# nlapier2/Metalign

Measured on NVIDIA B200. Metric: read k-mers/sec queried vs CMash DB, higher is better.
Workload: dtype u128

## Files before the change

metalign_b200/csrc/probe_mz.cu:

```cuda
#ifdef MZ_RT
#define MLG_RT MZ_RT
#endif
#include "probe_common.cuh"

namespace {

#ifndef MZ_MINCTAS
#define MZ_MINCTAS 2
#endif
constexpr unsigned MZ_MAXRUN = 4;
constexpr unsigned MZ_QDRAIN = 32;
constexpr unsigned MZ_QCAP = MZ_QDRAIN + 128;
constexpr unsigned MZ_LIST = 16;
constexpr uint32_t MZ_M64 = MLG_MZ_ORD_MULT << 6;
#ifndef MZ_TILE_READS
#define MZ_TILE_READS 32
#endif
constexpr unsigned MZ_TR = MZ_TILE_READS;
static_assert(MZ_TR % 32 == 0 && MZ_TR >= 32 && MZ_TR <= 128, "tile = whole warp passes");
constexpr unsigned MZ_STAGE_B = MZ_TR * 40 + 64;
constexpr unsigned MZ_STAGE_M = MZ_TR * 20 + 64;
struct MzStage {
    __align__(16) unsigned char b[WARPS][2][MZ_STAGE_B];
    __align__(16) unsigned char m[WARPS][2][MZ_STAGE_M];
};
struct MzShared {
    MzStage stg;
    uint32_t wm[MZ_LIST][RT];
    uint32_t seq[SEGW + 1][RT];
    uint32_t qa[WARPS][MZ_QCAP];
    uint32_t qc[WARPS][MZ_QCAP];
    uint32_t qb[WARPS][MZ_QCAP];
    uint32_t qoff[WARPS][32];
    uint32_t qn[WARPS];
};
constexpr uint32_t MZ_ROW = RT * 4;

#ifndef MZ_L2_FETCH
#define MZ_L2_FETCH 64
#endif
#if MZ_L2_FETCH == 64
#define MZ_L2Q ".L2::64B"
#elif MZ_L2_FETCH == 128
#define MZ_L2Q ".L2::128B"
#else
#define MZ_L2Q ""
#endif
__device__ __forceinline__ uint32_t ldg_bitmap_if(bool p, const uint32_t* ptr) {
    uint32_t r;
    asm volatile(
        "{\n"
        ".reg .pred q;\n"
        "setp.ne.u32 q, %1, 0;\n"
        "mov.u32 %0, 0;\n"
        "@q ld.global.nc.L1::no_allocate" MZ_L2Q ".b32 %0, [%2];\n"
        "}\n" : "=r"(r) : "r"((uint32_t)p), "l"(ptr));
    return r;
}
__device__ __forceinline__ uint32_t ldg_u32(const uint32_t* ptr) {
    uint32_t r;
    asm volatile("ld.global.nc" MZ_L2Q ".b32 %0, [%1];" : "=r"(r) : "l"(ptr));
    return r;
}
__device__ __forceinline__ key128 ldg_key(const key128* ptr) {
    key128 k;
    asm volatile("ld.global.nc" MZ_L2Q ".v2.u64 {%0, %1}, [%2];" : "=l"(k.hi), "=l"(k.lo) : "l"(ptr));
    return k;
}
template <bool HAS_NMASK>
__device__ __forceinline__ void segment_load_staged(uint32_t (&loc)[SEGW], uint32_t (&nl)[5], uint32_t brel, uint32_t mrel, uint32_t sb, uint32_t sk) {
    const uint32_t ab = sb + (brel >> 4) * 4u;
    const unsigned sh = 2u * (brel & 15u);
    uint32_t W[SEGW + 1];
#pragma unroll
    for (int k = 0; k <= (int)SEGW; ++k) W[k] = __byte_perm(lds32(ab + 4u * (uint32_t)k), 0, 0x0123);
#pragma unroll
    for (int k = 0; k < (int)SEGW; ++k) loc[k] = fsl(W[k], W[k + 1], sh);
#pragma unroll
    for (int k = 0; k < 5; ++k) nl[k] = 0;
    if (HAS_NMASK) {
        const uint32_t am = sk + (mrel >> 5) * 4u;
        const unsigned shn = mrel & 31u;
        uint32_t M[6];
#pragma unroll
        for (int k = 0; k < 6; ++k) M[k] = __byte_perm(lds32(am + 4u * (uint32_t)k), 0, 0x0123);
#pragma unroll
        for (int k = 0; k < 5; ++k) nl[k] = fsl(M[k], M[k + 1], shn);
    }
}
__device__ __forceinline__ uint32_t mz_val(const uint32_t (&loc)[SEGW], const uint32_t (&rcl)[SEGW], int j, int i) {
    const uint32_t a = fsl(loc[j], loc[j + 1], 2 * i);
    const int ra = i <= 11 ? 7 - j : 6 - j, ro = i <= 11 ? 11 - i : 27 - i;
    const uint32_t b = fsl(rcl[ra], rcl[ra + 1], 2 * ro);
    return b * MZ_M64 + (a * MZ_M64 + (uint32_t)(16 * j + i));
}
__device__ __forceinline__ void mz_bases64(const unsigned long long* bsrc, unsigned long long base_words, unsigned long long p,
                                           unsigned long long& hi, unsigned long long& lo) {
    const unsigned long long q = p >> 5;
    const unsigned sh = 2u * (unsigned)(p & 31ull);
    unsigned long long W[3];
#pragma unroll
    for (int k = 0; k < 3; ++k) {
        unsigned long long idx = q + k;
        if (idx >= base_words) idx = base_words - 1;
        W[k] = bswap64(bsrc[idx]);
    }
    hi = sh ? ((W[0] << sh) | (W[1] >> (64 - sh))) : W[0];
    lo = sh ? ((W[1] << sh) | (W[2] >> (64 - sh))) : W[1];
}
struct MzWin {
    key128 cn, d0, d1;
    uint32_t s, e, j0, j1;
};
__device__ __forceinline__ void mz_window_begin(MzWin& w, bool on, unsigned long long p, unsigned long long pm,
                                                const unsigned long long* bsrc, unsigned long long base_words, const DbView& db) {
    w.s = w.e = w.j0 = w.j1 = 0;
    w.cn.hi = w.cn.lo = 0; w.d0 = w.cn; w.d1 = w.cn;
    if (!on) return;
    key128 F;
    mz_bases64(bsrc, base_words, p, F.hi, F.lo);
    const unsigned dsh = 2u * (unsigned)(pm - p);
    const unsigned long long mh = dsh ? ((F.hi << dsh) | (F.lo >> (64u - dsh))) : F.hi;
    const uint32_t ha = (uint32_t)(mh >> 32), hb = rev2_32(~(uint32_t)mh);
    const uint32_t zhi = mz_ident_hi(ha, hb), zlo = mz_ident_lo(ha, hb);
    const uint32_t bucket = zhi >> (32u - db.bbits);
    w.s = ldg_u32(db.bstart + bucket); w.e = ldg_u32(db.bstart + bucket + 1);
    if (db.n_alias && ((db.alias_bloom[(zlo & 0xFFFFu) >> 5] >> (zlo & 31u)) & 1u)) {
        const unsigned long long z = ((unsigned long long)zhi << 32) | zlo;
        uint32_t lo = 0, hi = db.n_alias;
        while (lo < hi) { const uint32_t mid = (lo + hi) >> 1; if (db.alias_z[mid] < z) lo = mid + 1; else hi = mid; }
        w.j0 = w.j1 = lo;
        while (w.j1 < db.n_alias && db.alias_z[w.j1] == z) ++w.j1;
    }
    F = key_shr(F, 128 - 2 * SK_K);
    const key128 G = key_rc(F, SK_K);
    w.cn = key_lt(G, F) ? G : F;
    if (w.s < w.e) w.d0 = ldg_key(db.D_key + w.s);
    if (w.s + 1u < w.e) w.d1 = ldg_key(db.D_key + w.s + 1u);
}
__device__ __forceinline__ void mz_window_end(const MzWin& w, const DbView& db, const CountSink& cs) {
    if (w.s < w.e && w.d0.hi == w.cn.hi && w.d0.lo == w.cn.lo) { bump_counter(cs, w.s); return; }
    if (w.s + 1u < w.e && w.d1.hi == w.cn.hi && w.d1.lo == w.cn.lo) { bump_counter(cs, w.s + 1u); return; }
    for (uint32_t i = w.s + 2u; i < w.e; ++i) {
        const key128 d = ldg_key(db.D_key + i);
        if (d.hi == w.cn.hi && d.lo == w.cn.lo) { bump_counter(cs, i); return; }
    }
    for (uint32_t j = w.j0; j < w.j1; ++j) {
        const uint32_t i = db.alias_i[j];
        const key128 d = db.D_key[i];
        if (d.hi == w.cn.hi && d.lo == w.cn.lo) { bump_counter(cs, i); return; }
    }
}
__device__ __noinline__ void mz_drain(uint32_t* qn, const uint32_t* qa, const uint32_t* qc, uint32_t* qb, uint32_t* qoff,
                                      const ProbeArgs& a, const DbView& db) {
    const unsigned long long* const bsrc = a.bases;
    const unsigned long long base_words = a.base_words;
    const CountSink cs{a.cnt8, a.present, a.n_present, a.touched, a.ci_min};
    constexpr unsigned FULL = 0xFFFFFFFFu;
    const unsigned lane = threadIdx.x & 31u;
    __syncwarp();
    const uint32_t n = *qn;
    for (uint32_t base = 0; base < n; base += 32u) {
        const uint32_t i = base + lane;
        uint32_t kb0 = i < n ? qb[i] : 0u;
        if (__any_sync(FULL, (kb0 >> 31) != 0u)) {
            if (kb0 >> 31) {
                const unsigned long long pb = ((unsigned long long)qc[i] << 32) | qa[i];
                unsigned long long mh, ml;
                mz_bases64(bsrc, base_words, pb + ((kb0 >> 16) & 63u), mh, ml);
                const uint32_t ha = (uint32_t)(mh >> 32), hb = rev2_32(~(uint32_t)mh);
                const uint32_t zhi = mz_ident_hi(ha, hb), zlo = mz_ident_lo(ha, hb);
                const unsigned long long idx = mz_bit_index(((unsigned long long)zhi << 32) | zlo, db.fbits);
                const uint32_t f = ldg_u32(db.F + (idx >> 5));
                kb0 = ((f >> (zlo & 31u)) & (f >> mz_bit2(zhi)) & 1u) ? (kb0 & 0x7FFFFFFFu) : 0u;
                qb[i] = kb0;
            }
            __syncwarp();
        }
        const uint32_t cnt = (uint32_t)__popc(kb0 & 0xFFFFu);
        uint32_t inc = cnt;
#pragma unroll
        for (int o = 1; o < 32; o <<= 1) { const uint32_t u = __shfl_up_sync(FULL, inc, o); if ((int)lane >= o) inc += u; }
        const uint32_t total = __shfl_sync(FULL, inc, 31);
        qoff[lane] = inc - cnt;
        __syncwarp();
        for (uint32_t w = lane; w < total; w += 32u) {
            uint32_t j = 0;
#pragma unroll
            for (uint32_t step = 16; step; step >>= 1) if (qoff[j + step] <= w) j += step;
            const uint32_t kb = qb[base + j];
            const uint32_t tt = __fns(kb & 0xFFFFu, 0u, (int)(w - qoff[j]) + 1);
            const unsigned long long pb = ((unsigned long long)qc[base + j] << 32) | qa[base + j];
            MzWin win;
            mz_window_begin(win, true, pb + tt, pb + ((kb >> 16) & 63u), bsrc, base_words, db);
            mz_window_end(win, db, cs);
        }
        __syncwarp();
    }
    __syncwarp();
    if (lane == 0) *qn = 0;
    __syncwarp();
}

template <bool HAS_NMASK>
__global__ void __launch_bounds__(RT, MZ_MINCTAS) k1_minimizer_probe(const __grid_constant__ ProbeArgs a, const __grid_constant__ DbView db) {
    extern __shared__ __align__(16) unsigned char smem_raw[];
    MzShared& sm = *reinterpret_cast<MzShared*>(smem_raw);
    MzStage& stg = sm.stg;
    __shared__ __align__(8) unsigned long long mbar[WARPS][2];
    __shared__ unsigned long long s_bw0[WARPS][2], s_mw0[WARPS][2];
    __shared__ unsigned s_staged[WARPS][2];
    __shared__ __align__(16) uint32_t s_zero[SEGW + 2];

    const unsigned tid = threadIdx.x, warp = tid >> 5, lane = tid & 31u;
    constexpr unsigned K = SK_K;
    if (tid < SEGW + 2) s_zero[tid] = 0u;
    constexpr unsigned FULL = 0xFFFFFFFFu;
    const unsigned long long nreads = a.r_end - a.r_begin;
    const unsigned long long ntiles = (nreads + MZ_TR - 1) / MZ_TR;
    unsigned int* const tile_ctr = reinterpret_cast<unsigned int*>(a.tile_counter);
    auto next_tile = [&]() -> unsigned long long {
        unsigned int t = 0;
        if (lane == 0) t = atomicAdd(tile_ctr, 1u);
        return __shfl_sync(FULL, t, 0);
    };
#ifdef MZ_STREAM_EVICT_FIRST
    const unsigned long long pol_stream = policy_evict_first();
#elif defined(MZ_STREAM_EVICT_LAST)
    const unsigned long long pol_stream = policy_evict_last();
#else
    unsigned long long pol_stream;
    asm volatile("createpolicy.fractional.L2::evict_normal.b64 %0, 1.0;" : "=l"(pol_stream));
#endif
    const uint32_t wm_base = smem_u32(&sm.wm[0][tid]), seq_base = smem_u32(&sm.seq[0][tid]);
    const uint32_t* const MB = db.F;
    const uint32_t lt_mask = (1u << lane) - 1u;
    const uint32_t fmask_lo = db.fbits >= 32u ? 0xFFFFFFFFu : ((1u << db.fbits) - 1u);
    const uint32_t fmask_hi = db.fbits > 32u ? ((1u << (db.fbits - 32u)) - 1u) : 0u;

    if (lane == 0) {
        mbar_init(&mbar[warp][0], 1);
        mbar_init(&mbar[warp][1], 1);
        asm volatile("fence.mbarrier_init.release.cluster;" ::: "memory");
    }
    __syncthreads();

    auto issue = [&](unsigned stage, unsigned long long t) {
        const unsigned long long r0 = a.r_begin + t * (unsigned long long)MZ_TR;
        const unsigned long long r1 = (r0 + MZ_TR < a.r_end) ? r0 + MZ_TR : a.r_end;
        const unsigned long long p0 = a.off ? a.off[r0] : r0 * (unsigned long long)a.read_len;
        const unsigned long long p1 = a.off ? a.off[r1] : r1 * (unsigned long long)a.read_len;
        unsigned long long bw0 = (p0 >> 5) & ~1ull;
        unsigned long long bw1 = ((p1 + 31) >> 5) + 6;
        if (bw1 > a.base_words) bw1 = a.base_words;
        bw1 = (bw1 + 1) & ~1ull;
        unsigned long long mw0 = (p0 >> 6) & ~1ull;
        unsigned long long mw1 = ((p1 + 63) >> 6) + 4;
        if (HAS_NMASK) { if (mw1 > a.nmask_words) mw1 = a.nmask_words; mw1 = (mw1 + 1) & ~1ull; }
        const unsigned long long bytes_b = (bw1 - bw0) * 8ull, bytes_m = HAS_NMASK ? (mw1 - mw0) * 8ull : 0ull;
        const bool fits = bw1 > bw0 && bytes_b <= MZ_STAGE_B && bytes_m <= MZ_STAGE_M;
        s_bw0[warp][stage] = bw0; s_mw0[warp][stage] = mw0; s_staged[warp][stage] = fits ? 1u : 0u;
        if (fits) {
            mbar_expect_tx(&mbar[warp][stage], (uint32_t)(bytes_b + bytes_m));
            bulk_g2s(&stg.b[warp][stage][0], a.bases + bw0, (uint32_t)bytes_b, &mbar[warp][stage], pol_stream);
            if (HAS_NMASK && bytes_m) bulk_g2s(&stg.m[warp][stage][0], a.nmask + mw0, (uint32_t)bytes_m, &mbar[warp][stage], pol_stream);
        } else {
            mbar_arrive(&mbar[warp][stage]);
        }
    };

    unsigned my_valid = 0;
    unsigned my_fetch = 0;
    if (lane == 0) sm.qn[warp] = 0;
    __syncwarp();

    auto halves_at = [&](uint32_t P, uint32_t& ha, uint32_t& hb) {
        const uint32_t ad = seq_base + (P >> 4) * MZ_ROW;
        const uint32_t w0 = lds32(ad), w1 = lds32(ad + MZ_ROW), w2 = lds32(ad + 2u * MZ_ROW);
        const unsigned sh = 2u * (P & 15u);
        ha = fsl(w0, w1, sh);
        hb = rev2_32(~fsl(w1, w2, sh));
    };
    auto drain = [&]() {
        mz_drain(&sm.qn[warp], &sm.qa[warp][0], &sm.qc[warp][0], &sm.qb[warp][0], &sm.qoff[warp][0], a, db);
    };
    auto push = [&](bool p, unsigned long long pb, uint32_t ik, uint32_t rel) {
        if (p) {
            const uint32_t i = atomicAdd(&sm.qn[warp], 1u);
            sm.qa[warp][i] = (uint32_t)pb; sm.qc[warp][i] = (uint32_t)(pb >> 32); sm.qb[warp][i] = ik | (rel << 16);
        }
    };
    auto drain_if_full = [&]() {
        __syncwarp();
        if (sm.qn[warp] >= MZ_QDRAIN) drain();
    };

    unsigned it = 0;
    unsigned long long t = next_tile(), t_ahead = next_tile();
    if (lane == 0) {
        if (t < ntiles) issue(0, t);
        if (t_ahead < ntiles) issue(1, t_ahead);
    }
    for (; t < ntiles; ++it) {
        const unsigned stage = it & 1u, parity = (it >> 1) & 1u;
        __syncwarp();
        mbar_wait(&mbar[warp][stage], parity);

        const bool staged = s_staged[warp][stage] != 0;
        const unsigned long long bw0_32 = s_bw0[warp][stage] * 32ull, mw0_64 = s_mw0[warp][stage] * 64ull;
        const uint32_t sb_stage = smem_u32(&stg.b[warp][stage][0]), sk_stage = smem_u32(&stg.m[warp][stage][0]), s_zero_a = smem_u32(&s_zero[0]);
#pragma unroll 1
        for (unsigned half = 0; half < MZ_TR / 32u; ++half) {
        const unsigned long long r = a.r_begin + t * (unsigned long long)MZ_TR + half * 32u + lane;
        if (half && r - lane >= a.r_end) break;
        const bool active = r < a.r_end;
        unsigned long long R0 = 0, R1 = 0;
        if (active) {
            R0 = a.off ? a.off[r] : r * (unsigned long long)a.read_len;
            R1 = a.off ? a.off[r + 1] : R0 + a.read_len;
        }
        const unsigned long long len = R1 - R0;
        const unsigned long long nw = len >= K ? len - K + 1 : 0ull;
        const unsigned nseg = (unsigned)((nw + WMAX - 1) / WMAX);
        const unsigned max_seg = __reduce_max_sync(FULL, nseg);
        const uint32_t brel0 = (uint32_t)(R0 - bw0_32), mrel0 = (uint32_t)(R0 - mw0_64);
        __syncwarp();

        for (unsigned seg = 0; seg < max_seg; ++seg) {
            const unsigned c = seg < nseg ? (unsigned)((nw - (unsigned long long)seg * WMAX) < WMAX ? (nw - (unsigned long long)seg * WMAX) : WMAX) : 0u;
            const unsigned long long s = bw0_32 + brel0 + (unsigned long long)seg * WMAX;

            uint32_t loc[SEGW];
            uint32_t nl[5];
            if (staged) segment_load_staged<HAS_NMASK>(loc, nl, c ? brel0 + seg * WMAX : 0u, c ? mrel0 + seg * WMAX : 0u, c ? sb_stage : s_zero_a, c ? sk_stage : s_zero_a);
            else segment_load<HAS_NMASK>(loc, nl, c, s, a.bases, a.nmask, a.base_words, a.nmask_words);
            uint32_t v0, v1, v2;
            segment_valid<HAS_NMASK>(nl, c, K, v0, v1, v2);
            my_valid += __popc(v0) + __popc(v1) + __popc(v2);
            if (__all_sync(FULL, (v0 | v1 | v2) == 0u)) continue;

#pragma unroll
            for (int k = 0; k < (int)SEGW; ++k) sts32(seq_base + (uint32_t)k * MZ_ROW, loc[k]);
            sts32(seq_base + SEGW * MZ_ROW, 0u);

            uint32_t rcl[SEGW];
            segment_rc60(loc, rcl);

            uint32_t P = 0xFFFFFFFFu;
#pragma unroll
            for (int i = 0; i < 12; ++i) P = min(P, mz_val(loc, rcl, 1, i));
            uint32_t held_wm = 0;
            bool have = false, held_pass = false;

            bool pend = false, pneed0 = false, more = true;
            uint32_t pW = 0, pchg = 0, pvm = 0, pnr = 0, pblk = 0;
            uint32_t pX0 = 0, pX1 = 0, pX2 = 0, pX3 = 0, pbits = 0, pbit2 = 0;
#pragma unroll 1
            for (int blk = 0;; ++blk) {
                const uint32_t blk16 = (uint32_t)blk * 16u;
                uint32_t F0 = 0, F1 = 0, F2 = 0, F3 = 0;
                if (pend) {
                    F0 = ldg_bitmap_if(pneed0, MB + pX0);
                    F1 = ldg_bitmap_if(pnr > 1u, MB + pX1);
                    F2 = ldg_bitmap_if(pnr > 2u, MB + pX2);
                    F3 = ldg_bitmap_if(pnr > 3u, MB + pX3);
                    my_fetch += (pneed0 ? 1u : 0u) + pnr - 1u;
                }
                uint32_t chgraw = 0, wm_first = 0, vb = 0;
                if (more) {
                    vb = v0 & 0xFFFF0000u;
                    v0 = fsl(v0, v1, 16); v1 = fsl(v1, v2, 16); v2 <<= 16;
                    uint32_t Suf[16];
                    {
                        uint32_t smn = 0xFFFFFFFFu;
#pragma unroll
                        for (int i = 15; i >= 0; --i) { smn = min(smn, mz_val(loc, rcl, 0, i)); Suf[i] = smn; }
                    }
                    uint32_t A1 = 0, pw = 0;
                    uint32_t lst = wm_base + MZ_ROW;
#pragma unroll
                    for (int tt = 0; tt < 16; ++tt) {
                        uint32_t wm;
                        if (tt < 4) {
                            P = min(P, mz_val(loc, rcl, 1, 12 + tt));
                            wm = min(Suf[tt], P);
                            if (tt == 3) { A1 = P; P = 0xFFFFFFFFu; }
                        } else {
                            P = min(P, mz_val(loc, rcl, 2, tt - 4));
                            wm = min(min(Suf[tt], A1), P);
                        }
                        if (tt == 0) wm_first = wm;
                        else if (wm != pw) {
                            sts32(lst, wm);
                            lst += MZ_ROW;
                            chgraw |= 1u << tt;
                        }
                        pw = wm;
                    }
                    P -= 16u;
                }
                bool nneed0 = false;
                uint32_t nW = 0, nchg = 0, nvm = 0, nnr = 1, nX0 = 0, nX1 = 0, nX2 = 0, nX3 = 0, nbits = 0, nbit2 = 0;
                if (more) {
                    uint32_t t3 = chgraw;
                    t3 &= t3 - 1u; t3 &= t3 - 1u; t3 &= t3 - 1u;
                    nchg = chgraw ^ t3;
                    const uint32_t ovfm = t3 ? (~((t3 & (0u - t3)) - 1u) & 0xFFFFu) : 0u;
                    const uint32_t vwin = __brev(vb) & 0xFFFFu;
                    nnr = 1u + __popc(nchg);
                    nvm = vwin & ~ovfm;
                    if (__any_sync(FULL, t3 != 0u)) {
                        const unsigned long long ia = s_bw0[warp][stage] * 32ull + brel0 + (unsigned long long)seg * WMAX + blk16;
                        uint32_t rest = t3;
                        unsigned rr = MZ_MAXRUN;
                        while (__any_sync(FULL, rest != 0u)) {
                            const uint32_t low = rest & (0u - rest), nxt = rest ^ low;
                            const uint32_t upto = nxt ? (nxt & (0u - nxt)) : 0x10000u;
                            const uint32_t mk = rest ? ((upto - low) & vwin) : 0u;
                            const uint32_t w = rest ? lds32(wm_base + rr * MZ_ROW) : 0u;
                            push(mk != 0u, ia, mk, (w & 63u) | 0x8000u);
                            drain_if_full();
                            rest = nxt; ++rr;
                        }
                    }
                    const uint32_t W1 = lds32(wm_base + 1u * MZ_ROW), W2 = lds32(wm_base + 2u * MZ_ROW), W3 = lds32(wm_base + 3u * MZ_ROW);
                    nneed0 = !have || wm_first != held_wm;
                    have = true;
                    held_wm = (nnr == 1u ? wm_first : nnr == 2u ? W1 : nnr == 3u ? W2 : W3) - 16u;
                    nW = (wm_first & 63u) | ((W1 & 63u) << 8) | ((W2 & 63u) << 16) | ((W3 & 63u) << 24);
                    auto locate = [&](uint32_t w, unsigned sl) -> uint32_t {
                        uint32_t ha, hb;
                        halves_at(blk16 + (w & 63u), ha, hb);
                        const uint32_t zlo = mz_ident_lo(ha, hb) & fmask_lo, zhi = mz_ident_hi(ha, hb);
                        nbits |= (zlo & 31u) << (8u * sl);
                        nbit2 |= mz_bit2(zhi) << (8u * sl);
                        return (zlo >> 5) | ((zhi & fmask_hi) << 27);
                    };
                    nX0 = locate(wm_first, 0); nX1 = locate(W1, 1); nX2 = locate(W2, 2); nX3 = locate(W3, 3);
                }
                if (pend) {
                    auto both = [&](uint32_t f, unsigned sh) -> bool {
                        return ((f >> ((pbits >> sh) & 31u)) & (f >> ((pbit2 >> sh) & 31u)) & 1u) != 0u;
                    };
                    const bool b0 = pneed0 ? both(F0, 0) : held_pass;
                    const bool b1 = (pnr > 1u) & both(F1, 8);
                    const bool b2 = (pnr > 2u) & both(F2, 16);
                    const bool b3 = (pnr > 3u) & both(F3, 24);
                    held_pass = pnr == 1u ? b0 : pnr == 2u ? b1 : pnr == 3u ? b2 : b3;
                    if (__any_sync(FULL, b0 | b1 | b2 | b3)) {
                        uint32_t cc = pchg | 0x70000u;
                        const uint32_t c1 = cc & (0u - cc); cc ^= c1;
                        const uint32_t c2 = cc & (0u - cc); cc ^= c2;
                        const uint32_t c3 = cc & (0u - cc);
                        const uint32_t m0 = (c1 - 1u) & pvm, m1 = (c2 - c1) & pvm, m2 = (c3 - c2) & pvm, m3 = (0x10000u - c3) & pvm;
                        const bool q0 = b0 & (m0 != 0u), q1 = b1 & (m1 != 0u), q2 = b2 & (m2 != 0u), q3 = b3 & (m3 != 0u);
                        const unsigned long long ia = s_bw0[warp][stage] * 32ull + brel0 + (unsigned long long)seg * WMAX + pblk;
                        push(q0, ia, m0, pW & 63u);
                        push(q1, ia, m1, (pW >> 8) & 63u);
                        push(q2, ia, m2, (pW >> 16) & 63u);
                        push(q3, ia, m3, pW >> 24);
                        drain_if_full();
                    }
                }
                if (!more) break;
                pneed0 = nneed0; pW = nW; pnr = nnr; pchg = nchg; pvm = nvm; pblk = blk16; pend = true;
                pX0 = nX0; pX1 = nX1; pX2 = nX2; pX3 = nX3; pbits = nbits; pbit2 = nbit2;
                more = blk + 1 < (int)(WMAX / 16) && !__all_sync(FULL, (v0 | v1 | v2) == 0u);
#pragma unroll
                for (int k = 0; k < (int)SEGW - 1; ++k) loc[k] = loc[k + 1];
#pragma unroll
                for (int k = (int)SEGW - 1; k > 0; --k) rcl[k] = rcl[k - 1];
            }
        }
        }
        __syncwarp();
        const unsigned long long t_new = next_tile();
        if (lane == 0 && t_new < ntiles) issue(stage, t_new);
        t = t_ahead; t_ahead = t_new;
    }

    drain();
    unsigned long long warp_valid = my_valid;
    for (int o = 16; o > 0; o >>= 1) warp_valid += __shfl_down_sync(FULL, warp_valid, o);
    my_fetch = __reduce_add_sync(FULL, my_fetch);
    if (lane == 0 && warp_valid) atomicAdd(a.n_kmers, warp_valid);
    if (lane == 0 && my_fetch) atomicAdd(a.n_kmers + 1, (unsigned long long)my_fetch);
}

constexpr size_t K1MZ_SMEM = sizeof(MzShared);

template <bool HAS_NMASK>
int launch_mz_t(const DbView& db, const ProbeArgs& a, cudaStream_t st, unsigned grid) {
    auto kern = k1_minimizer_probe<HAS_NMASK>;
    static bool done[64] = {};
    int dev = 0;
    CUDA_TRY(cudaGetDevice(&dev));
    if (dev < 0 || dev >= 64 || !done[dev]) {
        CUDA_TRY(cudaFuncSetAttribute(kern, cudaFuncAttributeMaxDynamicSharedMemorySize, (int)K1MZ_SMEM));
        if (const char* e = getenv("MLG_PROBE_CARVEOUT")) { int x = atoi(e); if (x >= 0 && x <= 100) CUDA_TRY(cudaFuncSetAttribute(kern, cudaFuncAttributePreferredSharedMemoryCarveout, x)); }
        if (dev >= 0 && dev < 64) done[dev] = true;
    }
    CUDA_TRY(cudaMemsetAsync(a.tile_counter, 0, 8, st));
    kern<<<grid, RT, K1MZ_SMEM, st>>>(a, db);
    CUDA_TRY(cudaGetLastError());
    return MLG_OK;
}

}

int launch_probe_mz(const DbView& db, const ProbeArgs& a, cudaStream_t st, int sm_count) {
    if (db.K != SK_K || !db.F) { mlg_set_error("minimizer-bitmap layout needs K=60 and its bit array"); return MLG_ERR_STATE; }
    const unsigned long long wtiles = (a.r_end - a.r_begin + MZ_TR - 1) / MZ_TR;
    const unsigned long long need = (wtiles + WARPS - 1) / WARPS;
    int per_sm = MZ_MINCTAS;
    if (const char* e = getenv("MLG_PROBE_CTAS_PER_SM")) { int x = atoi(e); if (x >= 1 && x <= 64) per_sm = x; }
    const unsigned long long res = (unsigned long long)sm_count * (unsigned)per_sm;
    const unsigned grid = (unsigned)(need < res ? need : res);
    return a.nmask ? launch_mz_t<true>(db, a, st, grid) : launch_mz_t<false>(db, a, st, grid);
}
```

Measured before the change: 381.0 billion.

## Split minimizer scan and bitmap probing into separate batched phases

Restructures the per-segment loop into two passes. The first computes window minimizers for all blocks and records run starts as byte offsets in shared memory plus change bitmasks. The second probes the filter bitmap in groups of four independent loads, so more memory requests are in flight per warp. This replaces the old one-block-ahead software pipeline with its held-minimizer reuse, and overflow runs beyond a cap fall back to a scalar recompute. It adds shared-memory byte stores, extra bookkeeping and possibly redundant fetches, because a minimizer shared across block boundaries is no longer reused.

```diff
diff --git a/metalign_b200/csrc/probe_mz.cu b/metalign_b200/csrc/probe_mz.cu
--- a/metalign_b200/csrc/probe_mz.cu
+++ b/metalign_b200/csrc/probe_mz.cu
@@ -8,10 +8,11 @@
 #ifndef MZ_MINCTAS
 #define MZ_MINCTAS 2
 #endif
-constexpr unsigned MZ_MAXRUN = 4;
+constexpr unsigned MZ_LGROUP = 4;
 constexpr unsigned MZ_QDRAIN = 32;
 constexpr unsigned MZ_QCAP = MZ_QDRAIN + 128;
-constexpr unsigned MZ_LIST = 16;
+constexpr unsigned MZ_LIST = 64;
+constexpr unsigned MZ_CAP = MZ_LIST - 16;
 constexpr uint32_t MZ_M64 = MLG_MZ_ORD_MULT << 6;
 #ifndef MZ_TILE_READS
 #define MZ_TILE_READS 32
@@ -26,7 +27,7 @@
 };
 struct MzShared {
     MzStage stg;
-    uint32_t wm[MZ_LIST][RT];
+    unsigned char rl[MZ_LIST][RT];
     uint32_t seq[SEGW + 1][RT];
     uint32_t qa[WARPS][MZ_QCAP];
     uint32_t qc[WARPS][MZ_QCAP];
@@ -60,6 +61,12 @@
 __device__ __forceinline__ uint32_t ldg_u32(const uint32_t* ptr) {
     uint32_t r;
     asm volatile("ld.global.nc" MZ_L2Q ".b32 %0, [%1];" : "=r"(r) : "l"(ptr));
+    return r;
+}
+__device__ __forceinline__ void sts8(uint32_t addr, uint32_t v) { asm volatile("st.shared.u8 [%0], %1;" ::"r"(addr), "r"(v) : "memory"); }
+__device__ __forceinline__ uint32_t lds8(uint32_t addr) {
+    uint32_t r;
+    asm volatile("ld.shared.u8 %0, [%1];" : "=r"(r) : "r"(addr));
     return r;
 }
 __device__ __forceinline__ key128 ldg_key(const key128* ptr) {
@@ -232,7 +239,7 @@
     unsigned long long pol_stream;
     asm volatile("createpolicy.fractional.L2::evict_normal.b64 %0, 1.0;" : "=l"(pol_stream));
 #endif
-    const uint32_t wm_base = smem_u32(&sm.wm[0][tid]), seq_base = smem_u32(&sm.seq[0][tid]);
+    const uint32_t rl_base = smem_u32(&sm.rl[0][tid]), seq_base = smem_u32(&sm.seq[0][tid]);
     const uint32_t* const MB = db.F;
     const uint32_t lt_mask = (1u << lane) - 1u;
     const uint32_t fmask_lo = db.fbits >= 32u ? 0xFFFFFFFFu : ((1u << db.fbits) - 1u);
@@ -349,127 +356,132 @@
             uint32_t P = 0xFFFFFFFFu;
 #pragma unroll
             for (int i = 0; i < 12; ++i) P = min(P, mz_val(loc, rcl, 1, i));
-            uint32_t held_wm = 0;
-            bool have = false, held_pass = false;
-
-            bool pend = false, pneed0 = false, more = true;
-            uint32_t pW = 0, pchg = 0, pvm = 0, pnr = 0, pblk = 0;
-            uint32_t pX0 = 0, pX1 = 0, pX2 = 0, pX3 = 0, pbits = 0, pbit2 = 0;
+            const int lastv = v2 ? 96 - __ffs(v2) : v1 ? 64 - __ffs(v1) : v0 ? 32 - __ffs(v0) : -1;
+            const unsigned nblk = __reduce_max_sync(FULL, (unsigned)(lastv + 16) >> 4);
+            uint32_t pw = 0xFFFFFFFFu;
+            uint32_t lst = rl_base;
+            uint32_t c0 = 0, c1 = 0, c2 = 0;
 #pragma unroll 1
-            for (int blk = 0;; ++blk) {
-                const uint32_t blk16 = (uint32_t)blk * 16u;
-                uint32_t F0 = 0, F1 = 0, F2 = 0, F3 = 0;
-                if (pend) {
-                    F0 = ldg_bitmap_if(pneed0, MB + pX0);
-                    F1 = ldg_bitmap_if(pnr > 1u, MB + pX1);
-                    F2 = ldg_bitmap_if(pnr > 2u, MB + pX2);
-                    F3 = ldg_bitmap_if(pnr > 3u, MB + pX3);
-                    my_fetch += (pneed0 ? 1u : 0u) + pnr - 1u;
+            for (unsigned blk = 0; blk < nblk; ++blk) {
+                lst = min(lst, rl_base + MZ_CAP * RT);
+                uint32_t Suf[16];
+                {
+                    uint32_t smn = 0xFFFFFFFFu;
+#pragma unroll
+                    for (int i = 15; i >= 0; --i) { smn = min(smn, mz_val(loc, rcl, 0, i)); Suf[i] = smn; }
                 }
-                uint32_t chgraw = 0, wm_first = 0, vb = 0;
-                if (more) {
-                    vb = v0 & 0xFFFF0000u;
-                    v0 = fsl(v0, v1, 16); v1 = fsl(v1, v2, 16); v2 <<= 16;
-                    uint32_t Suf[16];
-                    {
-                        uint32_t smn = 0xFFFFFFFFu;
-#pragma unroll
-                        for (int i = 15; i >= 0; --i) { smn = min(smn, mz_val(loc, rcl, 0, i)); Suf[i] = smn; }
+                uint32_t A1 = 0, chg = 0;
+#pragma unroll
+                for (int tt = 0; tt < 16; ++tt) {
+                    uint32_t wm;
+                    if (tt < 4) {
+                        P = min(P, mz_val(loc, rcl, 1, 12 + tt));
+                        wm = min(Suf[tt], P);
+                        if (tt == 3) { A1 = P; P = 0xFFFFFFFFu; }
+                    } else {
+                        P = min(P, mz_val(loc, rcl, 2, tt - 4));
+                        wm = min(min(Suf[tt], A1), P);
                     }
-                    uint32_t A1 = 0, pw = 0;
-                    uint32_t lst = wm_base + MZ_ROW;
-#pragma unroll
-                    for (int tt = 0; tt < 16; ++tt) {
-                        uint32_t wm;
-                        if (tt < 4) {
-                            P = min(P, mz_val(loc, rcl, 1, 12 + tt));
-                            wm = min(Suf[tt], P);
-                            if (tt == 3) { A1 = P; P = 0xFFFFFFFFu; }
-                        } else {
-                            P = min(P, mz_val(loc, rcl, 2, tt - 4));
-                            wm = min(min(Suf[tt], A1), P);
-                        }
-                        if (tt == 0) wm_first = wm;
-                        else if (wm != pw) {
-                            sts32(lst, wm);
-                            lst += MZ_ROW;
-                            chgraw |= 1u << tt;
-                        }
-                        pw = wm;
+                    if (wm != pw) {
+                        sts8(lst, wm);
+                        lst += RT;
+                        chg |= 1u << tt;
                     }
-                    P -= 16u;
+                    pw = wm;
                 }
-                bool nneed0 = false;
-                uint32_t nW = 0, nchg = 0, nvm = 0, nnr = 1, nX0 = 0, nX1 = 0, nX2 = 0, nX3 = 0, nbits = 0, nbit2 = 0;
-                if (more) {
-                    uint32_t t3 = chgraw;
-                    t3 &= t3 - 1u; t3 &= t3 - 1u; t3 &= t3 - 1u;
-                    nchg = chgraw ^ t3;
-                    const uint32_t ovfm = t3 ? (~((t3 & (0u - t3)) - 1u) & 0xFFFFu) : 0u;
-                    const uint32_t vwin = __brev(vb) & 0xFFFFu;
-                    nnr = 1u + __popc(nchg);
-                    nvm = vwin & ~ovfm;
-                    if (__any_sync(FULL, t3 != 0u)) {
-                        const unsigned long long ia = s_bw0[warp][stage] * 32ull + brel0 + (unsigned long long)seg * WMAX + blk16;
-                        uint32_t rest = t3;
-                        unsigned rr = MZ_MAXRUN;
-                        while (__any_sync(FULL, rest != 0u)) {
-                            const uint32_t low = rest & (0u - rest), nxt = rest ^ low;
-                            const uint32_t upto = nxt ? (nxt & (0u - nxt)) : 0x10000u;
-                            const uint32_t mk = rest ? ((upto - low) & vwin) : 0u;
-                            const uint32_t w = rest ? lds32(wm_base + rr * MZ_ROW) : 0u;
-                            push(mk != 0u, ia, mk, (w & 63u) | 0x8000u);
-                            drain_if_full();
-                            rest = nxt; ++rr;
-                        }
-                    }
-                    const uint32_t W1 = lds32(wm_base + 1u * MZ_ROW), W2 = lds32(wm_base + 2u * MZ_ROW), W3 = lds32(wm_base + 3u * MZ_ROW);
-                    nneed0 = !have || wm_first != held_wm;
-                    have = true;
-                    held_wm = (nnr == 1u ? wm_first : nnr == 2u ? W1 : nnr == 3u ? W2 : W3) - 16u;
-                    nW = (wm_first & 63u) | ((W1 & 63u) << 8) | ((W2 & 63u) << 16) | ((W3 & 63u) << 24);
-                    auto locate = [&](uint32_t w, unsigned sl) -> uint32_t {
+                P -= 16u;
+                pw -= 16u;
+                c0 = __funnelshift_r(c0, c1, 16); c1 = __funnelshift_r(c1, c2, 16); c2 = __funnelshift_r(c2, chg, 16);
+#pragma unroll
+                for (int k = 0; k < (int)SEGW - 1; ++k) loc[k] = loc[k + 1];
+#pragma unroll
+                for (int k = (int)SEGW - 1; k > 0; --k) rcl[k] = rcl[k - 1];
+            }
+            for (unsigned blk = nblk; blk < WMAX / 16u; ++blk) { c0 = __funnelshift_r(c0, c1, 16); c1 = __funnelshift_r(c1, c2, 16); c2 >>= 16; }
+
+            {
+                const uint32_t lim = (uint32_t)(lastv + 1);
+                c0 &= lim >= 32u ? 0xFFFFFFFFu : (1u << lim) - 1u;
+                c1 &= lim >= 64u ? 0xFFFFFFFFu : lim > 32u ? (1u << (lim - 32u)) - 1u : 0u;
+                c2 &= lim >= 96u ? 0xFFFFFFFFu : lim > 64u ? (1u << (lim - 64u)) - 1u : 0u;
+            }
+            const uint32_t nr = (uint32_t)(__popc(c0) + __popc(c1) + __popc(c2));
+            uint32_t fw = 0;
+            c0 = __funnelshift_r(c0, c1, 1); c1 = __funnelshift_r(c1, c2, 1); c2 >>= 1;
+            auto next_start = [&]() -> uint32_t {
+                const uint32_t d = __ffs(c0);
+                c0 = __funnelshift_r(c0, c1, d); c1 = __funnelshift_r(c1, c2, d); c2 >>= d;
+                return d ? fw + d : WMAX;
+            };
+            const uint32_t V0 = __brev(v0), V1 = __brev(v1), V2 = __brev(v2);
+            auto emit = [&](bool on, uint32_t pk, uint32_t unt) {
+                const uint32_t f = pk & 127u, e = (pk >> 8) & 127u, pz = pk >> 16;
+                const unsigned long long ia = s_bw0[warp][stage] * 32ull + brel0 + (unsigned long long)seg * WMAX;
+#pragma unroll
+                for (uint32_t k = 0; k < 3u; ++k) {
+                    const uint32_t b0 = (f & ~15u) + 16u * k;
+                    const uint32_t vb = ((b0 < 32u ? V0 : b0 < 64u ? V1 : V2) >> (b0 & 16u)) & 0xFFFFu;
+                    const uint32_t lo = k == 0 ? f - b0 : 0u, hi = e < b0 + 16u ? e - b0 : 16u;
+                    const uint32_t mk = e > b0 ? (0xFFFFu << lo) & (0xFFFFu >> (16u - hi)) & vb : 0u;
+                    push(on && mk != 0u, ia + b0, mk, (pz - b0) | unt);
+                }
+            };
+
+            const uint32_t nrc = min(nr, MZ_CAP);
+            const uint32_t nmax = __reduce_max_sync(FULL, nrc);
+#pragma unroll 1
+            for (uint32_t i0 = 0; i0 < nmax; i0 += MZ_LGROUP) {
+                uint32_t Fw[MZ_LGROUP], Bt[MZ_LGROUP], Pk[MZ_LGROUP];
+#pragma unroll
+                for (uint32_t g = 0; g < MZ_LGROUP; ++g) {
+                    Fw[g] = 0; Bt[g] = 0; Pk[g] = 0;
+                    if (i0 + g < nmax) {
+                        const bool on = i0 + g < nrc;
+                        const uint32_t nx = next_start();
+                        const uint32_t pz = on ? (fw & ~15u) + (lds8(rl_base + (i0 + g) * RT) & 63u) : 0u;
                         uint32_t ha, hb;
-                        halves_at(blk16 + (w & 63u), ha, hb);
+                        halves_at(pz, ha, hb);
                         const uint32_t zlo = mz_ident_lo(ha, hb) & fmask_lo, zhi = mz_ident_hi(ha, hb);
-                        nbits |= (zlo & 31u) << (8u * sl);
-                        nbit2 |= mz_bit2(zhi) << (8u * sl);
-                        return (zlo >> 5) | ((zhi & fmask_hi) << 27);
-                    };
-                    nX0 = locate(wm_first, 0); nX1 = locate(W1, 1); nX2 = locate(W2, 2); nX3 = locate(W3, 3);
-                }
-                if (pend) {
-                    auto both = [&](uint32_t f, unsigned sh) -> bool {
-                        return ((f >> ((pbits >> sh) & 31u)) & (f >> ((pbit2 >> sh) & 31u)) & 1u) != 0u;
-                    };
-                    const bool b0 = pneed0 ? both(F0, 0) : held_pass;
-                    const bool b1 = (pnr > 1u) & both(F1, 8);
-                    const bool b2 = (pnr > 2u) & both(F2, 16);
-                    const bool b3 = (pnr > 3u) & both(F3, 24);
-                    held_pass = pnr == 1u ? b0 : pnr == 2u ? b1 : pnr == 3u ? b2 : b3;
-                    if (__any_sync(FULL, b0 | b1 | b2 | b3)) {
-                        uint32_t cc = pchg | 0x70000u;
-                        const uint32_t c1 = cc & (0u - cc); cc ^= c1;
-                        const uint32_t c2 = cc & (0u - cc); cc ^= c2;
-                        const uint32_t c3 = cc & (0u - cc);
-                        const uint32_t m0 = (c1 - 1u) & pvm, m1 = (c2 - c1) & pvm, m2 = (c3 - c2) & pvm, m3 = (0x10000u - c3) & pvm;
-                        const bool q0 = b0 & (m0 != 0u), q1 = b1 & (m1 != 0u), q2 = b2 & (m2 != 0u), q3 = b3 & (m3 != 0u);
-                        const unsigned long long ia = s_bw0[warp][stage] * 32ull + brel0 + (unsigned long long)seg * WMAX + pblk;
-                        push(q0, ia, m0, pW & 63u);
-                        push(q1, ia, m1, (pW >> 8) & 63u);
-                        push(q2, ia, m2, (pW >> 16) & 63u);
-                        push(q3, ia, m3, pW >> 24);
-                        drain_if_full();
+                        Bt[g] = (zlo & 31u) | (mz_bit2(zhi) << 8);
+                        Fw[g] = ldg_bitmap_if(on, MB + ((zlo >> 5) | ((zhi & fmask_hi) << 27)));
+                        Pk[g] = fw | (nx << 8) | (pz << 16);
+                        my_fetch += on ? 1u : 0u;
+                        fw = nx;
                     }
                 }
-                if (!more) break;
-                pneed0 = nneed0; pW = nW; pnr = nnr; pchg = nchg; pvm = nvm; pblk = blk16; pend = true;
-                pX0 = nX0; pX1 = nX1; pX2 = nX2; pX3 = nX3; pbits = nbits; pbit2 = nbit2;
-                more = blk + 1 < (int)(WMAX / 16) && !__all_sync(FULL, (v0 | v1 | v2) == 0u);
-#pragma unroll
-                for (int k = 0; k < (int)SEGW - 1; ++k) loc[k] = loc[k + 1];
-#pragma unroll
-                for (int k = (int)SEGW - 1; k > 0; --k) rcl[k] = rcl[k - 1];
+                uint32_t pm = 0;
+#pragma unroll
+                for (uint32_t g = 0; g < MZ_LGROUP; ++g) pm |= ((Fw[g] >> (Bt[g] & 31u)) & (Fw[g] >> (Bt[g] >> 8)) & 1u) << g;
+                while (__any_sync(FULL, pm != 0u)) {
+                    const uint32_t g = __ffs(pm) - 1u;
+                    uint32_t pk = Pk[0];
+#pragma unroll
+                    for (uint32_t h = 1; h < MZ_LGROUP; ++h) if (g == h) pk = Pk[h];
+                    emit(pm != 0u, pk, 0u);
+                    pm &= pm - 1u;
+                    drain_if_full();
+                }
+            }
+            if (__any_sync(FULL, nr > MZ_CAP)) {
+#pragma unroll 1
+                for (uint32_t i = MZ_CAP; __any_sync(FULL, i < nr); ++i) {
+                    const bool on = i < nr;
+                    const uint32_t nx = next_start();
+                    uint32_t pk = 0;
+                    if (on) {
+                        uint32_t best = 0xFFFFFFFFu;
+#pragma unroll 1
+                        for (uint32_t q = 0; q + MLG_MZ_M <= K; ++q) {
+                            uint32_t ha, hb;
+                            halves_at(fw + q, ha, hb);
+                            best = min(best, (ha + hb) * MZ_M64 + q);
+                        }
+                        pk = fw | (nx << 8) | ((fw + (best & 63u)) << 16);
+                    }
+                    emit(on, pk, 0x8000u);
+                    drain_if_full();
+                    fw = nx;
+                }
             }
         }
         }
```

New measurement: 419.3 billion, median of 6. 1.1x the previous value.
